# chenghuige/golden-huffman

Hardware: AMD Instinct MI355X
Metric: encode+decode GB/s (input bytes) (higher is better)
Workload: dtype u8

## Files before the change

### golden-huffman_amd/csrc/ghf_kernels.hip

```cpp
#include "ghf_device.h"

namespace ghf {

#define GHF_HADD(x, sh) atomicAdd(&lh[((((x) >> (sh)) & 0xFFu) << 5) | rep], 1u)

__device__ __forceinline__ void hist_vec(uint32_t* lh, uint32_t rep, const uint4& v) {
  GHF_HADD(v.x, 0); GHF_HADD(v.x, 8); GHF_HADD(v.x, 16); GHF_HADD(v.x, 24);
  GHF_HADD(v.y, 0); GHF_HADD(v.y, 8); GHF_HADD(v.y, 16); GHF_HADD(v.y, 24);
  GHF_HADD(v.z, 0); GHF_HADD(v.z, 8); GHF_HADD(v.z, 16); GHF_HADD(v.z, 24);
  GHF_HADD(v.w, 0); GHF_HADD(v.w, 8); GHF_HADD(v.w, 16); GHF_HADD(v.w, 24);
}

__global__ __launch_bounds__(kHistThreads) void k_histogram(const uint8_t* __restrict__ in, uint64_t n,
                                                            uint32_t chunk32, uint32_t nchunks,
                                                            uint32_t* __restrict__ chunk_hist,
                                                            unsigned long long* __restrict__ hist,
                                                            unsigned long long* __restrict__ acc ,
                                                            uint32_t add ) {
  static_assert(kHistRep == 32, "replica index is lane % 32");
  __shared__ uint32_t lh[256 * kHistRep];
  __shared__ bool s_last;
  const uint32_t tid = threadIdx.x;
  const uint32_t rep = tid & 31u;
  uint32_t prev = 0;
  unsigned long long total = 0;
  const uint64_t chunk = chunk32;
  const uint32_t V = chunk32 >> 12;
  const uint32_t nfullchunks = (uint32_t)(n / chunk);
  const bool fast = V >= 4u && (chunk32 & 4095u) == 0 && (((uintptr_t)in) & 15u) == 0 && nfullchunks > 0;
  auto vptr = [&](uint32_t c, uint32_t j) -> const uint4* {
    if (c >= nfullchunks) c = nfullchunks - 1;
    return reinterpret_cast<const uint4*>(in + (uint64_t)c * chunk) + (uint64_t)j * kHistThreads + tid;
  };
  uint4 A = make_uint4(0, 0, 0, 0), B = A;
  if (fast) {
    A = load_stream(vptr(blockIdx.x, 0));
    B = load_stream(vptr(blockIdx.x, 1));
  }
  for (uint32_t i = tid; i < 256 * kHistRep; i += kHistThreads) lh[i] = 0;
  __syncthreads();

  __shared__ uint32_t s_tick;
  auto finish_chunk = [&](uint32_t c) -> uint32_t {
    __syncthreads();
    const uint32_t posted = s_tick;
    uint32_t s = 0;
#pragma unroll
    for (uint32_t j = 0; j < kHistRep; ++j) s += lh[(tid << 5) | ((j + tid) & 31u)];
    const uint32_t cnt = s - prev;
    prev = s;
    chunk_hist[(uint64_t)c * 256 + tid] = cnt;
    total += cnt;
    __syncthreads();
    return posted;
  };

  if (fast) {
    const uint32_t ncls = gridDim.x < 16u ? 1u : (gridDim.x < 128u ? gridDim.x >> 3 : 16u);
    const uint32_t cls = (blockIdx.x >> 3) % ncls;
    unsigned long long* tick = acc + 32 * 256 + 16 + cls * 16;
    auto draw = [&]() -> uint32_t { return 2u * gridDim.x + (uint32_t)atomicAdd(tick, 1ull) * ncls + cls; };
    uint32_t cur = blockIdx.x;
    uint32_t nxt = blockIdx.x + gridDim.x;
    auto vat = [&](uint32_t g) -> const uint4* { return g < V ? vptr(cur, g) : vptr(nxt, g - V); };
    const uint32_t Vmain = V & ~3u, Vrest = V & 3u;
    while (cur < nfullchunks) {
      uint32_t t_next = 0;
      if (tid == 0) t_next = draw();
      for (uint32_t j = 0; j < Vmain; j += 4) {
        const uint4 C = load_stream(vat(j + 2)), D = load_stream(vat(j + 3));
        hist_vec(lh, rep, A);
        hist_vec(lh, rep, B);
        A = load_stream(vat(j + 4));
        B = load_stream(vat(j + 5));
        hist_vec(lh, rep, C);
        hist_vec(lh, rep, D);
      }
      if (Vrest == 1u) {
        hist_vec(lh, rep, A);
        A = B;
        B = load_stream(vptr(nxt, 1));
      } else if (Vrest == 2u) {
        hist_vec(lh, rep, A);
        hist_vec(lh, rep, B);
        A = load_stream(vptr(nxt, 0));
        B = load_stream(vptr(nxt, 1));
      } else if (Vrest == 3u) {
        const uint4 C = load_stream(vptr(cur, V - 1));
        hist_vec(lh, rep, A);
        hist_vec(lh, rep, B);
        A = load_stream(vptr(nxt, 0));
        B = load_stream(vptr(nxt, 1));
        hist_vec(lh, rep, C);
      }
      if (tid == 0) s_tick = t_next;
      const uint32_t posted = finish_chunk(cur);
      cur = nxt;
      nxt = posted;
    }
  }

  const uint32_t g0 = fast ? (blockIdx.x == 0 ? nfullchunks : nchunks) : blockIdx.x;
  const uint32_t gstep = fast ? nchunks : gridDim.x;
  for (uint32_t c = g0; c < nchunks; c += gstep) {
    const uint64_t base = (uint64_t)c * chunk;
    const uint64_t len = (n - base < chunk) ? (n - base) : chunk;
    const uint8_t* p = in + base;
    uint32_t head = (uint32_t)((16u - (uint32_t)((uintptr_t)p & 15u)) & 15u);
    if (head > len) head = (uint32_t)len;
    if (tid < head) atomicAdd(&lh[((uint32_t)p[tid] << 5) | rep], 1u);
    const uint4* pv = reinterpret_cast<const uint4*>(p + head);
    const uint64_t nvec = (len - head) >> 4;
    for (uint64_t i = tid; i < nvec; i += kHistThreads) {
      const uint4 v0 = pv[i];
      hist_vec(lh, rep, v0);
    }
    const uint64_t tail0 = head + (nvec << 4);
    if (tail0 + tid < len) atomicAdd(&lh[((uint32_t)p[tail0 + tid] << 5) | rep], 1u);
    (void)finish_chunk(c);
  }
  unsigned long long* rep_base = acc + (uint64_t)(blockIdx.x & 31u) * 256;
  if (total) atomicAdd(&rep_base[tid], total);
  asm volatile("s_waitcnt vmcnt(0)" ::: "memory");
  __syncthreads();
  if (tid == 0) {
    const unsigned long long t = atomicAdd(&acc[32 * 256], 1ull);
    s_last = (t + 1 == gridDim.x);
    if (s_last) __builtin_amdgcn_fence(__ATOMIC_ACQUIRE, "agent");
    asm volatile("s_waitcnt vmcnt(0)" ::: "memory");
  }
  __syncthreads();
  if (s_last) {
    unsigned long long part[32];
#pragma unroll
    for (int r = 0; r < 32; ++r) part[r] = __hip_atomic_load(&acc[r * 256 + tid], __ATOMIC_RELAXED, __HIP_MEMORY_SCOPE_AGENT);
    unsigned long long sum = 0;
#pragma unroll
    for (int r = 0; r < 32; ++r) {
      sum += part[r];
      __hip_atomic_store(&acc[r * 256 + tid], 0ull, __ATOMIC_RELAXED, __HIP_MEMORY_SCOPE_AGENT);
    }
    hist[tid] = add ? hist[tid] + sum : sum;
    if (tid < 16) __hip_atomic_store(&acc[32 * 256 + 16 + tid * 16], 0ull, __ATOMIC_RELAXED, __HIP_MEMORY_SCOPE_AGENT);
    if (tid == 0) {
      hist[256] = 1;
      __hip_atomic_store(&acc[32 * 256], 0ull, __ATOMIC_RELAXED, __HIP_MEMORY_SCOPE_AGENT);
    }
  }
}

void launch_histogram(const uint8_t* d_in, uint64_t n, uint32_t chunk, uint32_t nchunks, uint32_t* d_chunk_hist,
                      uint64_t* d_hist, uint64_t* d_acc, bool add, hipStream_t s) {
  static int ncu = 0;
  if (ncu == 0) {
    int dev = 0;
    hipDeviceProp_t prop;
    if (hipGetDevice(&dev) == hipSuccess && hipGetDeviceProperties(&prop, dev) == hipSuccess) ncu = prop.multiProcessorCount;
    if (ncu < 1) ncu = 256;
  }
  uint32_t grid = (uint32_t)(4 * ncu);
  if (grid > nchunks) grid = nchunks;
  if (grid == 0) grid = 1;
  hipLaunchKernelGGL(k_histogram, dim3(grid), dim3(kHistThreads), 0, s, d_in, n, chunk, nchunks, d_chunk_hist,
                     reinterpret_cast<unsigned long long*>(d_hist), reinterpret_cast<unsigned long long*>(d_acc),
                     add ? 1u : 0u);
}

struct HeapLds {
  alignas(16) unsigned long long slot[528];
  uint16_t parent[GHF_NSYM + 256 + 7];
  uint16_t cur[GHF_NSYM + 3];
};

typedef unsigned long long u64t;
struct alignas(16) U64x2 { u64t x, y; };

__device__ __forceinline__ bool heap_gt(u64t a, u64t b) { return a > (b | 511ull); }

__device__ __forceinline__ void heap_sift_up(HeapLds& h, int hole, u64t e) {
  while (hole > 0) {
    const int parent = (hole - 1) >> 1;
    const u64t pe = h.slot[parent + 1];
    if (!heap_gt(pe, e)) break;
    h.slot[hole + 1] = pe;
    hole = parent;
  }
  h.slot[hole + 1] = e;
}

__device__ __forceinline__ u64t heap_pop(HeapLds& h, int& n) {
  const u64t top = h.slot[1];
  const int len = n - 1;
  n = len;
  if (len < 1) return top;
  const u64t value = h.slot[len + 1];
  int hole = 0;
  const int lim = (len - 1) >> 1;
  while (hole < lim) {
    const U64x2 c = *reinterpret_cast<const U64x2*>(&h.slot[2 * hole + 2]);
    const U64x2 g0 = *reinterpret_cast<const U64x2*>(&h.slot[4 * hole + 4]);
    const U64x2 g1 = *reinterpret_cast<const U64x2*>(&h.slot[4 * hole + 6]);
    const bool left = heap_gt(c.y, c.x);
    const int child = 2 * hole + (left ? 1 : 2);
    h.slot[hole + 1] = left ? c.x : c.y;
    hole = child;
    if (hole < lim) {
      const U64x2 g = left ? g0 : g1;
      const bool left2 = heap_gt(g.y, g.x);
      const int child2 = 2 * hole + (left2 ? 1 : 2);
      h.slot[hole + 1] = left2 ? g.x : g.y;
      hole = child2;
    }
  }
  if ((len & 1) == 0 && hole == ((len - 2) >> 1)) {
    const int child = 2 * (hole + 1);
    h.slot[hole + 1] = h.slot[child];
    hole = child - 1;
  }
  heap_sift_up(h, hole, value);
  return top;
}

__device__ __forceinline__ u64t wave_uniform(u64t x) {
  const uint32_t lo = (uint32_t)__builtin_amdgcn_readfirstlane((int)(uint32_t)x);
  const uint32_t hi = (uint32_t)__builtin_amdgcn_readfirstlane((int)(uint32_t)(x >> 32));
  return ((u64t)hi << 32) | lo;
}

__device__ __forceinline__ u64t lane_above(u64t x) {
  const uint32_t lo = (uint32_t)__builtin_amdgcn_update_dpp(0, (int)(uint32_t)x, 0x101, 0xF, 0xF, false);
  const uint32_t hi = (uint32_t)__builtin_amdgcn_update_dpp(0, (int)(uint32_t)(x >> 32), 0x101, 0xF, 0xF, false);
  return ((u64t)hi << 32) | lo;
}

__device__ __forceinline__ u64t wave_heap_pop(HeapLds& h, int& n, int lane) {
  const int len = __builtin_amdgcn_readfirstlane(n) - 1;
  n = len;
  const uint32_t tA = lane ? (uint32_t)lane : 128u, tB = 64u + (uint32_t)lane;
  const U64x2 ca = *reinterpret_cast<const U64x2*>(&h.slot[2 * tA]);
  const U64x2 cb = *reinterpret_cast<const U64x2*>(&h.slot[2 * tB]);
  const u64t top_v = h.slot[1];
  const u64t value_v = h.slot[len + 1];
  __builtin_amdgcn_sched_barrier(0);
  const u64t top = wave_uniform(top_v);
  if (len < 1) return top;
  const u64t value = wave_uniform(value_v);
  const unsigned long long R0 = __ballot(!heap_gt(ca.y, ca.x));
  const unsigned long long R1 = __ballot(!heap_gt(cb.y, cb.x));
  const uint32_t lim = (uint32_t)(len - 1) >> 1;
  const int D = 31 - __clz(len);
  uint32_t t = 1;
  asm("s_bitcmp1_b64 %1, %0\n\ts_addc_u32 %0, %0, %0\n\t"
      "s_bitcmp1_b64 %1, %0\n\ts_addc_u32 %0, %0, %0\n\t"
      "s_bitcmp1_b64 %1, %0\n\ts_addc_u32 %0, %0, %0\n\t"
      "s_bitcmp1_b64 %1, %0\n\ts_addc_u32 %0, %0, %0\n\t"
      "s_bitcmp1_b64 %1, %0\n\ts_addc_u32 %0, %0, %0\n\t"
      "s_bitcmp1_b64 %1, %0\n\ts_addc_u32 %0, %0, %0\n\t"
      "s_bitcmp1_b64 %2, %0\n\ts_addc_u32 %0, %0, %0"
      : "+s"(t)
      : "s"(R0), "s"(R1)
      : "scc");
  const int steps = D - 1 > 0 ? D - 1 : 0;
  t >>= 7 - steps;
  if (t <= lim) t = 2u * t + (uint32_t)(((t < 64u || t == 128u ? R0 : R1) >> (t & 63u)) & 1ull);
  t <<= (((uint32_t)len & 1u) ^ 1u) & (uint32_t)(t == ((uint32_t)len >> 1));
  const int k = 31 - __clz(t);
  const uint32_t sh = (uint32_t)(k - lane) & 31u;
  const bool onp = lane < k;
  const uint32_t u = onp ? (t >> sh) : 1u;
  const U64x2 c = *reinterpret_cast<const U64x2*>(&h.slot[2 * u]);
  const u64t cv = ((t >> ((sh - 1u) & 31u)) & 1u) ? c.y : c.x;
  const unsigned long long S = __ballot(!heap_gt(cv, value)) & ((1ull << k) - 1ull);
  const int m = S ? 64 - __clzll((long long)S) : 0;
  if (lane <= m) h.slot[lane < m ? u : (t >> ((uint32_t)(k - m) & 31u))] = lane < m ? cv : value;
  wave_sync();
  return top;
}

struct PushLoad {
  u64t pe;
  int aj, depth;
  bool on;
};
__device__ __forceinline__ PushLoad wave_heap_push_load(const HeapLds& h, int n_, int lane) {
  const int n = __builtin_amdgcn_readfirstlane(n_);
  PushLoad L;
  L.depth = 31 - __clz(n + 1);
  L.on = lane >= 1 && lane <= L.depth;
  L.aj = ((n + 1) >> lane) - 1;
  L.pe = L.on ? h.slot[L.aj + 1] : 0ull;
  return L;
}
__device__ __forceinline__ void wave_heap_push_finish(HeapLds& h, const PushLoad& L, u64t e, int lane) {
  const bool stop = L.on && !heap_gt(L.pe, e);
  const unsigned long long sm = __ballot(stop);
  const int t = sm ? (__ffsll((long long)sm) - 1) - 1 : L.depth;
  const u64t up = lane_above(L.pe);
  if (lane <= t) h.slot[L.aj + 1] = (lane < t) ? up : e;
  wave_sync();
}
__device__ __forceinline__ void wave_heap_push(HeapLds& h, int n_, u64t e, int lane) {
  const PushLoad L = wave_heap_push_load(h, n_, lane);
  wave_heap_push_finish(h, L, e, lane);
}

struct CodeLds {
  uint32_t num[40];
  uint32_t first_code[64];
  uint32_t start_pos[64];
  int32_t min_len, max_len;
};

struct LimitLds {
  unsigned long long w[2][2 * GHF_NSYM];
  uint8_t is_leaf[33][2 * GHF_NSYM];
  uint16_t order[GHF_NSYM + 3];
  uint16_t len_of[34], taken[34];
  uint32_t newlen[GHF_NSYM + 3];
  long long freq[GHF_NSYM + 3];
  int n;
};

__device__ void limit_lengths_32(LimitLds& Q, const uint32_t (&len)[5], int lane) {
  constexpr int kLimit = 32;
  const long long* freq = Q.freq;
  if (lane == 0) Q.n = 0;
  __syncthreads();
#pragma unroll 1
  for (int j = 0; j < 5; ++j) {
    const int s = lane + 64 * j;
    if (s >= GHF_NSYM || len[j] == 0) continue;
    const long long f = freq[s];
    int rank = 0;
    for (int t = 0; t < GHF_NSYM; ++t) {
      const long long g = freq[t];
      rank += (g != 0) && (g < f || (g == f && t < s));
    }
    Q.order[rank] = (uint16_t)s;
    atomicAdd(&Q.n, 1);
  }
  __syncthreads();
  if (lane == 0) {
    const int n = Q.n;
    int prev_n = 0, cur = 0;
    for (int d = kLimit; d >= 1; --d) {
      const unsigned long long* pw = Q.w[cur ^ 1];
      unsigned long long* cw = Q.w[cur];
      const int npk = prev_n / 2;
      int li = 0, pi = 0, k = 0;
      while (li < n || pi < npk) {
        const unsigned long long lw = li < n ? (unsigned long long)freq[Q.order[li]] : ~0ull;
        const unsigned long long pk = pi < npk ? pw[2 * pi] + pw[2 * pi + 1] : ~0ull;
        if (li < n && (pi >= npk || lw <= pk)) {
          cw[k] = lw;
          Q.is_leaf[d][k] = 1;
          ++li;
        } else {
          cw[k] = pk;
          Q.is_leaf[d][k] = 0;
          ++pi;
        }
        ++k;
      }
      Q.len_of[d] = (uint16_t)k;
      prev_n = k;
      cur ^= 1;
    }
    int need = 2 * n - 2;
    for (int d = 1; d <= kLimit; ++d) {
      if (need > (int)Q.len_of[d]) need = Q.len_of[d];
      int leaves = 0;
      for (int k = 0; k < need; ++k) leaves += Q.is_leaf[d][k];
      Q.taken[d] = (uint16_t)leaves;
      need = 2 * (need - leaves);
    }
  }
  __syncthreads();
  for (int i = lane; i < GHF_NSYM; i += 64) Q.newlen[i] = 0;
  __syncthreads();
  for (int i = lane; i < Q.n; i += 64) {
    uint32_t l = 0;
    for (int d = 1; d <= kLimit; ++d) l += i < (int)Q.taken[d];
    Q.newlen[Q.order[i]] = l;
  }
  __syncthreads();
}

struct NoLimitLds {};
template <bool LIMIT>
__global__ __launch_bounds__(64) void k_build_code(const unsigned long long* __restrict__ hist, ghf_code* __restrict__ out,
                                                   int* __restrict__ status, uint32_t empty_ok) {
  __shared__ HeapLds heap;
  __shared__ typename std::conditional<LIMIT, LimitLds, NoLimitLds>::type Q;
  __builtin_amdgcn_s_setprio(3);
  __shared__ CodeLds cl;
  __shared__ int s_ndata;
  const int lane = threadIdx.x;
  long long fr[5];
#pragma unroll
  for (int j = 0; j < 5; ++j) {
    const int s = lane + 64 * j;
    fr[j] = s < GHF_NSYM ? (long long)hist[s] : 0ll;
    if constexpr (LIMIT) {
      if (s < GHF_NSYM) Q.freq[s] = fr[j];
    }
  }
  for (int s = lane; s < GHF_NSYM; s += 64) heap.cur[s] = (uint16_t)s;
  for (int i = lane; i < GHF_NSYM + 256 + 7; i += 64) heap.parent[i] = 0;
  if (lane < 40) cl.num[lane] = 0;
  cl.first_code[lane] = 0;
  cl.start_pos[lane] = 0;
  __syncthreads();

  {
    int n = 0, ndata = 0;
    for (int s = 0; s < GHF_NSYM; ++s) {
      const u64t f = (u64t)__shfl(fr[s >> 6], s & 63, 64);
      if (f) {
        wave_heap_push(heap, n, (f << 9) | (u64t)s, lane);
        ++n;
        if (s < 256) ++ndata;
      }
    }
    if (lane == 0) s_ndata = ndata;
    const int times = n - 1;
    for (int t = 0; t < times; ++t) {
      const u64t e1 = wave_heap_pop(heap, n, lane);
      const u64t e2 = wave_heap_pop(heap, n, lane);
      const int s1 = (int)(e1 & 511u), s2 = (int)(e2 & 511u);
      const int node = GHF_NSYM + t;
      const PushLoad pl = wave_heap_push_load(heap, n, lane);
      const uint16_t g1 = heap.cur[s1], g2 = heap.cur[s2];
      if (lane == 0) {
        heap.parent[g1] = (uint16_t)node;
        heap.parent[g2] = (uint16_t)node;
        heap.cur[s2] = (uint16_t)node;
      }
      const u64t f = (e1 >> 9) + (e2 >> 9);
      wave_heap_push_finish(heap, pl, (f << 9) | (u64t)s2, lane);
      ++n;
    }
  }
  __syncthreads();
  if (s_ndata == 0 && !empty_ok) {
    if (lane == 0) latch_status(status, GHF_E_EMPTY);
    return;
  }
  uint32_t len[5], node[5];
#pragma unroll
  for (int j = 0; j < 5; ++j) {
    len[j] = 0;
    node[j] = (uint32_t)(lane + 64 * j);
    if (node[j] >= GHF_NSYM) node[j] = GHF_NSYM + 256 + 1;
  }
  for (int step = 0; step < 256; ++step) {
    bool any = false;
#pragma unroll
    for (int j = 0; j < 5; ++j) {
      const uint32_t p = heap.parent[node[j]];
      if (p) {
        node[j] = p;
        len[j] += 1;
        any = true;
      }
    }
    if (!__ballot(any)) break;
  }
  if (s_ndata == 0 && lane == 0) len[4] = 1;
  uint32_t mx = 0;
#pragma unroll
  for (int j = 0; j < 5; ++j) {
    if (lane + 64 * j >= GHF_NSYM) len[j] = 0;
    mx = len[j] > mx ? len[j] : mx;
  }
#pragma unroll
  for (int d = 32; d >= 1; d >>= 1) {
    const uint32_t o = __shfl_xor(mx, d, 64);
    mx = o > mx ? o : mx;
  }
  int max_len = (int)mx;
  if (max_len > 32) {
    if constexpr (!LIMIT) {
      if (lane == 0) latch_status(status, GHF_E_CODELEN);
      return;
    } else {
      limit_lengths_32(Q, len, lane);
      mx = 0;
#pragma unroll
      for (int j = 0; j < 5; ++j) {
        const int s = lane + 64 * j;
        len[j] = s < GHF_NSYM ? Q.newlen[s] : 0u;
        mx = len[j] > mx ? len[j] : mx;
      }
#pragma unroll
      for (int d = 32; d >= 1; d >>= 1) {
        const uint32_t o = __shfl_xor(mx, d, 64);
        mx = o > mx ? o : mx;
      }
      max_len = (int)mx;
    }
  }

#pragma unroll
  for (int j = 0; j < 5; ++j) {
    const int s = lane + 64 * j;
    if (s < GHF_NSYM) {
      out->length[s] = len[j];
      out->codeword[s] = 0;
      out->symbol[s] = 0xFFFFFFFFu;
      if (len[j]) atomicAdd(&cl.num[len[j]], 1u);
    }
  }
  __syncthreads();
  const uint32_t num = (lane >= 1 && lane <= max_len) ? cl.num[lane] : 0u;
  const unsigned long long nzmask = __ballot(num != 0);
  const int min_len = __ffsll((long long)nzmask) - 1;
  const uint32_t spos = wave_incl_scan_u32(num) - num;
  if (lane >= 1 && lane <= max_len) cl.start_pos[lane] = spos;
  if (lane == 0) {
    uint32_t fc = 0;
    cl.first_code[max_len] = 0;
    for (int i = max_len - 1; i >= 1; --i) {
      fc = (fc + cl.num[i + 1]) >> 1;
      cl.first_code[i] = fc;
    }
    for (int i = 1; i < min_len; ++i) cl.first_code[i] = 1024;
    out->min_len = min_len;
    out->max_len = max_len;
  }
  __syncthreads();
  out->first_code[lane] = cl.first_code[lane];
  out->start_pos[lane] = cl.start_pos[lane];
  uint32_t seen = 0;
  for (int j = 0; j < 5; ++j) {
    for (int L = min_len; L <= max_len; ++L) {
      const bool m = (len[j] == (uint32_t)L);
      const unsigned long long mask = __ballot(m);
      if (mask == 0) continue;
      const uint32_t before = __shfl(seen, L, 64);
      if (m) {
        const uint32_t r = before + (uint32_t)__popcll(mask & ((1ull << lane) - 1ull));
        const int s = lane + 64 * j;
        out->codeword[s] = cl.first_code[L] + r;
        out->symbol[cl.start_pos[L] + r] = (uint32_t)s;
      }
      if (lane == L) seen += (uint32_t)__popcll(mask);
    }
  }
}

void launch_build_code(const uint64_t* d_hist, ghf_code* d_code, int* d_status, uint32_t flags, hipStream_t s) {
  if (flags & GHF_CODE_LIMIT)
    hipLaunchKernelGGL(k_build_code<true>, dim3(1), dim3(64), 0, s, reinterpret_cast<const unsigned long long*>(d_hist), d_code, d_status,
                       flags & GHF_EMPTY_OK);
  else
    hipLaunchKernelGGL(k_build_code<false>, dim3(1), dim3(64), 0, s, reinterpret_cast<const unsigned long long*>(d_hist), d_code, d_status,
                       flags & GHF_EMPTY_OK);
}

struct TreeLds {
  uint16_t tl[256], tr[256];
  uint16_t size[GHF_NSYM + 256 + 7];
  uint8_t is_right[GHF_NSYM + 256 + 7];
  uint32_t code_hi[256];
  uint32_t max_len, min_len;
  int n;
};

__global__ __launch_bounds__(64) void k_crs_build_code(const unsigned long long* __restrict__ hist, ghf_tree* __restrict__ out_tree,
                                                       ghf_code* __restrict__ out_code, unsigned long long* __restrict__ start_bit,
                                                       int* __restrict__ status) {
  __shared__ HeapLds heap;
  __shared__ TreeLds T;
  __shared__ ghf_tree tree;
  __builtin_amdgcn_s_setprio(3);
  const int lane = threadIdx.x;
  for (int s = lane; s < GHF_NSYM; s += 64) heap.cur[s] = (uint16_t)s;
  for (int i = lane; i < GHF_NSYM + 256 + 7; i += 64) {
    heap.parent[i] = 0;
    T.size[i] = 1;
    T.is_right[i] = 0;
  }
  for (int i = lane; i < (int)(sizeof(ghf_tree) / 4); i += 64) reinterpret_cast<uint32_t*>(&tree)[i] = 0;
  if (lane == 0) {
    T.max_len = 0;
    T.min_len = 0xFFFFFFFFu;
  }
  __syncthreads();
  int n = 0;
  for (int s = 0; s < 256; ++s) {
    const u64t f = wave_uniform((u64t)hist[s]);
    if (f) {
      wave_heap_push(heap, n, (f << 9) | (u64t)s, lane);
      ++n;
    }
  }
  const int nleaves = n;
  if (nleaves < 2) {
    if (lane == 0) latch_status(status, nleaves == 0 ? GHF_E_EMPTY : GHF_E_SINGLE);
    return;
  }
  const int times = n - 1;
  for (int t = 0; t < times; ++t) {
    const u64t e1 = wave_heap_pop(heap, n, lane);
    const u64t e2 = wave_heap_pop(heap, n, lane);
    const int s1 = (int)(e1 & 511u), s2 = (int)(e2 & 511u);
    const int node = GHF_NSYM + t;
    if (lane == 0) {
      const int a = heap.cur[s1], b = heap.cur[s2];
      heap.parent[a] = (uint16_t)node;
      heap.parent[b] = (uint16_t)node;
      T.tl[t] = (uint16_t)a;
      T.tr[t] = (uint16_t)b;
      T.is_right[b] = 1;
      T.size[node] = (uint16_t)(1 + T.size[a] + T.size[b]);
      heap.cur[s2] = (uint16_t)node;
    }
    wave_heap_push(heap, n, (((e1 >> 9) + (e2 >> 9)) << 9) | (u64t)s2, lane);
    ++n;
  }
  __syncthreads();
  for (int v = lane; v < GHF_NSYM + times; v += 64) {
    const bool leaf = v < 256;
    if (v == 256 || (leaf && heap.parent[v] == 0)) continue;
    uint32_t len = 0, pre = 0;
    unsigned long long code = 0;
    int x = v;
    for (int p; (p = heap.parent[x]) != 0; x = p) {
      const uint32_t r = T.is_right[x];
      if (len < 64) code |= (unsigned long long)r << len;
      ++len;
      pre += 1u + (r ? (uint32_t)T.size[T.tl[p - GHF_NSYM]] : 0u);
    }
    if (leaf) {
      tree.header[2 * pre] = 0;
      tree.header[2 * pre + 1] = (uint8_t)v;
      atomicMax(&T.max_len, len);
      atomicMin(&T.min_len, len);
      if (len <= 64) {
        out_code->length[v] = len;
        out_code->codeword[v] = (uint32_t)code;
        T.code_hi[v] = (uint32_t)(code >> 32);
      }
    } else {
      tree.header[2 * pre] = 255;
      tree.header[2 * pre + 1] = 255;
      const int t = v - GHF_NSYM;
      const int a = T.tl[t], b = T.tr[t];
      tree.left[t] = (uint16_t)(a < GHF_NSYM ? a : 256 + (a - GHF_NSYM));
      tree.right[t] = (uint16_t)(b < GHF_NSYM ? b : 256 + (b - GHF_NSYM));
    }
  }
  __syncthreads();
  const bool deep = T.max_len > 32u;
  for (int s = lane; s < GHF_NSYM; s += 64) {
    const bool absent = s == 256 || heap.parent[s] == 0;
    if (absent) {
      out_code->length[s] = 0;
      out_code->codeword[s] = 0;
    }
    out_code->symbol[s] = deep ? (absent ? 0u : T.code_hi[s]) : 0xFFFFFFFFu;
  }
  for (int i = lane; i < 64; i += 64) {
    out_code->first_code[i] = 0;
    out_code->start_pos[i] = 0;
  }
  if (T.max_len > 64u) {
    if (lane == 0) latch_status(status, GHF_E_CODELEN);
    return;
  }
  if (lane == 0) {
    tree.root = (uint32_t)(256 + times - 1);
    tree.n_leaves = (uint32_t)nleaves;
    tree.max_len = T.max_len;
    tree.tree_bytes = 2u * (2u * (uint32_t)nleaves - 1u);
    out_code->min_len = (int32_t)T.min_len;
    out_code->max_len = (int32_t)T.max_len;
    if (start_bit) *start_bit = 8ull * ((unsigned long long)tree.tree_bytes + 2ull);
  }
  __syncthreads();
  for (int i = lane; i < (int)(sizeof(ghf_tree) / 4); i += 64)
    reinterpret_cast<uint32_t*>(out_tree)[i] = reinterpret_cast<const uint32_t*>(&tree)[i];
}

void launch_crs_build_code(const uint64_t* d_hist, ghf_tree* d_tree, ghf_code* d_code, uint64_t* d_start_bit, int* d_status,
                           hipStream_t s) {
  hipLaunchKernelGGL(k_crs_build_code, dim3(1), dim3(64), 0, s, reinterpret_cast<const unsigned long long*>(d_hist), d_tree,
                     d_code, reinterpret_cast<unsigned long long*>(d_start_bit), d_status);
}

__global__ __launch_bounds__(256) void k_crs_finish(const ghf_tree* __restrict__ tree, const unsigned long long* __restrict__ total_bits,
                                                    uint8_t* __restrict__ out, unsigned long long* __restrict__ out_bytes,
                                                    const int* __restrict__ status) {
  if (*status != 0) return;
  const uint32_t tb = tree->tree_bytes;
  for (uint32_t i = threadIdx.x; i < tb; i += 256) out[i] = tree->header[i];
  if (threadIdx.x == 0) {
    const unsigned long long t = *total_bits;
    const unsigned long long whole = t >> 3;
    const uint32_t left = (uint32_t)((8u - (uint32_t)(t & 7u)) & 7u);
    out[tb] = (uint8_t)left;
    out[tb + 1] = left ? out[tb + 2 + whole] : (uint8_t)0;
    if (out_bytes) *out_bytes = (unsigned long long)tb + 2ull + whole;
  }
}

void launch_crs_finish(const ghf_tree* d_tree, const uint64_t* d_total_bits, uint8_t* d_out, uint64_t* d_out_bytes, int* d_status,
                       hipStream_t s) {
  hipLaunchKernelGGL(k_crs_finish, dim3(1), dim3(256), 0, s, d_tree, reinterpret_cast<const unsigned long long*>(d_total_bits), d_out,
                     reinterpret_cast<unsigned long long*>(d_out_bytes), d_status);
}

__global__ __launch_bounds__(256) void k_write_header(const ghf_code* __restrict__ code, uint8_t* __restrict__ out,
                                                      uint64_t cap, int* __restrict__ status) {
  const int max_len = code->max_len;
  if (max_len < 1 || max_len > 32) return;
  const int nwords = 1 + GHF_NSYM + 2 + 2 * max_len;
  if ((uint64_t)nwords * 4 > cap) {
    if (threadIdx.x == 0) latch_status(status, GHF_E_CAP);
    return;
  }
  uint32_t* o = reinterpret_cast<uint32_t*>(out);
  for (int w = threadIdx.x; w < nwords; w += blockDim.x) o[w] = bswap32(header_word(code, w, max_len));
}

void launch_write_header(const ghf_code* d_code, uint8_t* d_out, uint64_t cap, int* d_status, hipStream_t s) {
  hipLaunchKernelGGL(k_write_header, dim3(1), dim3(256), 0, s, d_code, d_out, cap, d_status);
}

__global__ __launch_bounds__(256) void k_chunk_bits(const uint32_t* __restrict__ chunk_hist, uint32_t nchunks,
                                                    const ghf_code* __restrict__ code, uint64_t* __restrict__ bits) {
  const int lane = threadIdx.x & 63;
  const uint32_t wave = (blockIdx.x * blockDim.x + threadIdx.x) >> 6;
  const uint32_t nwaves = (gridDim.x * blockDim.x) >> 6;
  const uint4 L = reinterpret_cast<const uint4*>(code->length)[lane];
  for (uint32_t c = wave; c < nchunks; c += nwaves) {
    const uint4 h = reinterpret_cast<const uint4*>(chunk_hist + (uint64_t)c * 256)[lane];
    unsigned long long b = (unsigned long long)h.x * L.x + (unsigned long long)h.y * L.y +
                           (unsigned long long)h.z * L.z + (unsigned long long)h.w * L.w;
#pragma unroll
    for (int d = 32; d >= 1; d >>= 1) b += __shfl_xor(b, d, 64);
    if (lane == 0) bits[c] = b;
  }
}

__global__ __launch_bounds__(256) void k_chunk_bits_direct(const uint8_t* __restrict__ in, uint64_t n, uint32_t chunk32,
                                                           uint32_t nchunks, const ghf_code* __restrict__ code,
                                                           uint64_t* __restrict__ bits) {
  __shared__ uint32_t ll[256];
  ll[threadIdx.x] = code->length[threadIdx.x];
  __syncthreads();
  const int lane = threadIdx.x & 63;
  const uint32_t wave = (blockIdx.x * blockDim.x + threadIdx.x) >> 6;
  const uint32_t nwaves = (gridDim.x * blockDim.x) >> 6;
  const uint64_t chunk = chunk32;
  for (uint32_t c = wave; c < nchunks; c += nwaves) {
    const uint64_t base = (uint64_t)c * chunk;
    const uint64_t len = (n - base < chunk) ? (n - base) : chunk;
    unsigned long long b = 0;
    const uint8_t* p = in + base;
    uint64_t head = (16u - (uint32_t)((uintptr_t)p & 15u)) & 15u;
    if (head > len) head = len;
    if ((uint64_t)lane < head) b += ll[p[lane]];
    const uint4* pv = reinterpret_cast<const uint4*>(p + head);
    const uint64_t nvec = (len - head) >> 4;
    uint32_t acc = 0;
    for (uint64_t i = lane; i < nvec; i += 64) {
      const uint4 v = pv[i];
      const uint32_t w[4] = {v.x, v.y, v.z, v.w};
#pragma unroll
      for (int k = 0; k < 4; ++k)
        acc += ll[w[k] & 0xFFu] + ll[(w[k] >> 8) & 0xFFu] + ll[(w[k] >> 16) & 0xFFu] + ll[w[k] >> 24];
      if ((i >> 6) % 4096u == 4095u) {
        b += acc;
        acc = 0;
      }
    }
    b += acc;
    const uint64_t tail0 = head + (nvec << 4);
    if (tail0 + (uint64_t)lane < len) b += ll[p[tail0 + lane]];
#pragma unroll
    for (int d = 32; d >= 1; d >>= 1) b += __shfl_xor(b, d, 64);
    if (lane == 0) bits[c] = b;
  }
}

__global__ __launch_bounds__(1024) void k_scan(uint64_t* __restrict__ v, uint32_t count, uint64_t* __restrict__ total_out) {
  __shared__ unsigned long long wsum[16];
  const int tid = threadIdx.x, lane = tid & 63, w = tid >> 6;
  const uint32_t ipt = (count + 1023u) / 1024u;
  const uint32_t lo = tid * ipt;
  const uint32_t hi = (lo + ipt < count) ? lo + ipt : count;
  unsigned long long mine = 0;
  const bool small = ipt <= 8u;
  unsigned long long x8[8];
  if (small) {
#pragma unroll
    for (uint32_t k = 0; k < 8; ++k) {
      const uint32_t i = lo + k;
      x8[k] = (k < ipt && i < hi) ? v[i] : 0ull;
    }
#pragma unroll
    for (uint32_t k = 0; k < 8; ++k) mine += x8[k];
  } else {
    for (uint32_t i = lo; i < hi; ++i) mine += v[i];
  }
  unsigned long long s = mine;
#pragma unroll
  for (int d = 1; d < 64; d <<= 1) {
    const unsigned long long t = __shfl_up(s, d, 64);
    if (lane >= d) s += t;
  }
  if (lane == 63) wsum[w] = s;
  __syncthreads();
  unsigned long long woff = 0, total = 0;
  for (int k = 0; k < 16; ++k) {
    const unsigned long long x = wsum[k];
    if (k < w) woff += x;
    total += x;
  }
  unsigned long long run = woff + s - mine;
  if (small) {
#pragma unroll
    for (uint32_t k = 0; k < 8; ++k) {
      const uint32_t i = lo + k;
      if (k < ipt && i < hi) v[i] = run;
      run += x8[k];
    }
  } else {
    for (uint32_t i = lo; i < hi; ++i) {
      const unsigned long long x = v[i];
      v[i] = run;
      run += x;
    }
  }
  if (tid == 0) {
    v[count] = total;
    if (total_out) *total_out = total;
  }
}

void launch_scan(uint64_t* d_v, uint32_t count, uint64_t* d_total, hipStream_t s) {
  hipLaunchKernelGGL(k_scan, dim3(1), dim3(1024), 0, s, d_v, count, d_total);
}

void launch_plan(const uint8_t* d_in, uint64_t n, uint32_t chunk, uint32_t nchunks, const uint32_t* d_chunk_hist,
                 const ghf_code* d_code, uint64_t* d_chunk_off, uint64_t* d_total_bits, hipStream_t s) {
  uint32_t blocks = (nchunks + 3) / 4;
  if (blocks > 2048) blocks = 2048;
  if (blocks == 0) blocks = 1;
  if (d_chunk_hist)
    hipLaunchKernelGGL(k_chunk_bits, dim3(blocks), dim3(256), 0, s, d_chunk_hist, nchunks, d_code, d_chunk_off);
  else
    hipLaunchKernelGGL(k_chunk_bits_direct, dim3(blocks), dim3(256), 0, s, d_in, n, chunk, nchunks, d_code,
                       d_chunk_off);
  hipLaunchKernelGGL(k_scan, dim3(1), dim3(1024), 0, s, d_chunk_off, nchunks, d_total_bits);
}

__global__ void k_store_u64(uint64_t* dst, const uint64_t* src, uint64_t add) { *dst = (src ? *src : 0ull) + add; }
void launch_store_u64(uint64_t* d_dst, const uint64_t* d_src_opt, uint64_t add, hipStream_t s) {
  hipLaunchKernelGGL(k_store_u64, dim3(1), dim3(1), 0, s, d_dst, d_src_opt, add);
}

__global__ void k_load_u16(uint64_t* dst, const uint16_t* src) { *dst = *src; }
void launch_load_u16(uint64_t* d_dst, const uint16_t* d_src, hipStream_t s) { hipLaunchKernelGGL(k_load_u16, dim3(1), dim3(1), 0, s, d_dst, d_src); }

__global__ void k_shard_start(const ghf_code* code, const uint64_t* totals, int rank, uint64_t* start_bit) {
  uint64_t b = 8ull * (1040ull + 8ull * (uint64_t)code->max_len);
  for (int r = 0; r < rank; ++r) b += totals[r];
  *start_bit = b;
}
void launch_shard_start(const ghf_code* d_code, const uint64_t* d_totals, int rank, uint64_t* d_start_bit, hipStream_t s) {
  hipLaunchKernelGGL(k_shard_start, dim3(1), dim3(1), 0, s, d_code, d_totals, rank, d_start_bit);
}

template <bool NT>
__global__ __launch_bounds__(256) void k_stream_copy(const uint4* __restrict__ src, uint4* __restrict__ dst, uint64_t nvec) {
  const uint64_t per = (nvec + gridDim.x - 1) / gridDim.x;
  const uint64_t lo = (uint64_t)blockIdx.x * per;
  const uint64_t end = lo + per < nvec ? lo + per : nvec;
  uint64_t i = lo + threadIdx.x;
  auto ld = [&](uint64_t k) -> uint4 { return NT ? load_stream(src + k) : src[k]; };
  auto st = [&](uint64_t k, const uint4& v) {
    if (NT) store_stream(dst + k, v);
    else dst[k] = v;
  };
  for (; i + 3 * 256 < end; i += 4 * 256) {
    const uint4 a = ld(i), b = ld(i + 256), c = ld(i + 512), d = ld(i + 768);
    st(i, a); st(i + 256, b); st(i + 512, c); st(i + 768, d);
  }
  for (; i < end; i += 256) st(i, ld(i));
}
__global__ void k_tail_copy(const uint8_t* src, uint8_t* dst, uint64_t from, uint64_t n) {
  const uint64_t i = from + threadIdx.x;
  if (i < n) dst[i] = src[i];
}
void launch_stream_copy(const uint8_t* d_src, uint8_t* d_dst, uint64_t n, bool nt, hipStream_t s) {
  const uint64_t nvec = n / 16;
  if (nvec) {
    uint64_t blocks = (nvec + 255) / 256;
    if (blocks > 4096) blocks = 4096;
    if (nt) hipLaunchKernelGGL(k_stream_copy<true>, dim3((uint32_t)blocks), dim3(256), 0, s, reinterpret_cast<const uint4*>(d_src), reinterpret_cast<uint4*>(d_dst), nvec);
    else hipLaunchKernelGGL(k_stream_copy<false>, dim3((uint32_t)blocks), dim3(256), 0, s, reinterpret_cast<const uint4*>(d_src), reinterpret_cast<uint4*>(d_dst), nvec);
  }
  if (n & 15) hipLaunchKernelGGL(k_tail_copy, dim3(1), dim3(16), 0, s, d_src, d_dst, nvec * 16, n);
}

}
```

Before: 965.8.

## Double-buffer histogram counts in 16-bit halves to drop a barrier per chunk

Each shared-memory histogram word now holds two 16-bit counters. Consecutive chunks alternate halves, so finish_chunk reads one half and clears it with atomicAnd while the next chunk accumulates into the other half. This removes the trailing __syncthreads and the running-prefix subtraction. The main loop also keeps four vectors in flight with sched_barrier fences, and the remainder cases are specialized at compile time. In exchange it adds an atomicAnd per replica and relies on a static_assert that a chunk's counts fit in 16 bits.

Result: no change. 962.4 (-0.4%).

```diff
diff --git a/golden-huffman_amd/csrc/ghf_kernels.hip b/golden-huffman_amd/csrc/ghf_kernels.hip
--- a/golden-huffman_amd/csrc/ghf_kernels.hip
+++ b/golden-huffman_amd/csrc/ghf_kernels.hip
@@ -2,14 +2,20 @@
 
 namespace ghf {
 
-#define GHF_HADD(x, sh) atomicAdd(&lh[((((x) >> (sh)) & 0xFFu) << 5) | rep], 1u)
-
-__device__ __forceinline__ void hist_vec(uint32_t* lh, uint32_t rep, const uint4& v) {
+static_assert(kMaxChunk / kHistRep + 2 * (kHistThreads / kHistRep) < 65536, "a chunk's counts must fit a 16-bit half");
+
+#define GHF_HADD(x, sh) atomicAdd(&lh[((((x) >> (sh)) & 0xFFu) << 5) | rep], inc)
+
+__device__ __forceinline__ void hist_vec(uint32_t* lh, uint32_t rep, uint32_t inc, const uint4& v) {
   GHF_HADD(v.x, 0); GHF_HADD(v.x, 8); GHF_HADD(v.x, 16); GHF_HADD(v.x, 24);
   GHF_HADD(v.y, 0); GHF_HADD(v.y, 8); GHF_HADD(v.y, 16); GHF_HADD(v.y, 24);
   GHF_HADD(v.z, 0); GHF_HADD(v.z, 8); GHF_HADD(v.z, 16); GHF_HADD(v.z, 24);
   GHF_HADD(v.w, 0); GHF_HADD(v.w, 8); GHF_HADD(v.w, 16); GHF_HADD(v.w, 24);
 }
+
+#define GHF_HFENCE() __builtin_amdgcn_sched_barrier(0)
+
+template <uint32_t N> struct HistRest { static constexpr uint32_t value = N; };
 
 __global__ __launch_bounds__(kHistThreads) void k_histogram(const uint8_t* __restrict__ in, uint64_t n,
                                                             uint32_t chunk32, uint32_t nchunks,
@@ -22,7 +28,7 @@
   __shared__ bool s_last;
   const uint32_t tid = threadIdx.x;
   const uint32_t rep = tid & 31u;
-  uint32_t prev = 0;
+  uint32_t half = 0;
   unsigned long long total = 0;
   const uint64_t chunk = chunk32;
   const uint32_t V = chunk32 >> 12;
@@ -32,71 +38,85 @@
     if (c >= nfullchunks) c = nfullchunks - 1;
     return reinterpret_cast<const uint4*>(in + (uint64_t)c * chunk) + (uint64_t)j * kHistThreads + tid;
   };
-  uint4 A = make_uint4(0, 0, 0, 0), B = A;
+  uint4 A = make_uint4(0, 0, 0, 0), B = A, C = A, D = A;
   if (fast) {
     A = load_stream(vptr(blockIdx.x, 0));
     B = load_stream(vptr(blockIdx.x, 1));
+    C = load_stream(vptr(blockIdx.x, 2));
+    D = load_stream(vptr(blockIdx.x, 3));
   }
   for (uint32_t i = tid; i < 256 * kHistRep; i += kHistThreads) lh[i] = 0;
   __syncthreads();
 
-  __shared__ uint32_t s_tick;
+  __shared__ uint32_t s_tick[2];
   auto finish_chunk = [&](uint32_t c) -> uint32_t {
     __syncthreads();
-    const uint32_t posted = s_tick;
+    const uint32_t posted = __builtin_amdgcn_readfirstlane(s_tick[half >> 4]);
+    const uint32_t keep = 0xFFFF0000u >> half;
     uint32_t s = 0;
 #pragma unroll
-    for (uint32_t j = 0; j < kHistRep; ++j) s += lh[(tid << 5) | ((j + tid) & 31u)];
-    const uint32_t cnt = s - prev;
-    prev = s;
-    chunk_hist[(uint64_t)c * 256 + tid] = cnt;
-    total += cnt;
-    __syncthreads();
+    for (uint32_t j = 0; j < kHistRep; ++j) {
+      uint32_t* p = &lh[(tid << 5) | ((j + tid) & 31u)];
+      s += (__hip_atomic_load(p, __ATOMIC_RELAXED, __HIP_MEMORY_SCOPE_WORKGROUP) >> half) & 0xFFFFu;
+      atomicAnd(p, keep);
+    }
+    chunk_hist[(uint64_t)c * 256 + tid] = s;
+    total += s;
+    half ^= 16u;
     return posted;
   };
 
   if (fast) {
     const uint32_t ncls = gridDim.x < 16u ? 1u : (gridDim.x < 128u ? gridDim.x >> 3 : 16u);
     const uint32_t cls = (blockIdx.x >> 3) % ncls;
-    unsigned long long* tick = acc + 32 * 256 + 16 + cls * 16;
-    auto draw = [&]() -> uint32_t { return 2u * gridDim.x + (uint32_t)atomicAdd(tick, 1ull) * ncls + cls; };
-    uint32_t cur = blockIdx.x;
-    uint32_t nxt = blockIdx.x + gridDim.x;
-    auto vat = [&](uint32_t g) -> const uint4* { return g < V ? vptr(cur, g) : vptr(nxt, g - V); };
-    const uint32_t Vmain = V & ~3u, Vrest = V & 3u;
-    while (cur < nfullchunks) {
-      uint32_t t_next = 0;
-      if (tid == 0) t_next = draw();
-      for (uint32_t j = 0; j < Vmain; j += 4) {
-        const uint4 C = load_stream(vat(j + 2)), D = load_stream(vat(j + 3));
-        hist_vec(lh, rep, A);
-        hist_vec(lh, rep, B);
-        A = load_stream(vat(j + 4));
-        B = load_stream(vat(j + 5));
-        hist_vec(lh, rep, C);
-        hist_vec(lh, rep, D);
+    uint32_t* tick = reinterpret_cast<uint32_t*>(acc + 32 * 256 + 16 + cls * 16);
+    const uint32_t Vmain = V & ~3u;
+    auto fast_chunks = [&](auto rest) {
+      constexpr uint32_t R = decltype(rest)::value;
+      uint32_t cur = blockIdx.x;
+      uint32_t nxt = blockIdx.x + gridDim.x;
+      auto vat = [&](uint32_t j, uint32_t k) -> const uint4* {
+        return j + 4 < Vmain ? vptr(cur, j + 4 + k) : vptr(nxt, k);
+      };
+      uint4 E0 = A, E1 = A, E2 = A;
+      while (cur < nfullchunks) {
+        uint32_t drawn = 0;
+        if (tid == 0) drawn = atomicAdd(tick, 1u);
+        const uint32_t inc = 1u << half;
+        if (R >= 1u) E0 = load_stream(vptr(cur, Vmain));
+        if (R >= 2u) E1 = load_stream(vptr(cur, Vmain + 1));
+        if (R >= 3u) E2 = load_stream(vptr(cur, Vmain + 2));
+        GHF_HFENCE();
+        uint32_t j = 0;
+        do {
+          hist_vec(lh, rep, inc, A);
+          hist_vec(lh, rep, inc, B);
+          GHF_HFENCE();
+          A = load_stream(vat(j, 0));
+          B = load_stream(vat(j, 1));
+          GHF_HFENCE();
+          hist_vec(lh, rep, inc, C);
+          hist_vec(lh, rep, inc, D);
+          GHF_HFENCE();
+          C = load_stream(vat(j, 2));
+          D = load_stream(vat(j, 3));
+          GHF_HFENCE();
+          j += 4;
+        } while (j < Vmain);
+        if (R >= 1u) hist_vec(lh, rep, inc, E0);
+        if (R >= 2u) hist_vec(lh, rep, inc, E1);
+        if (R >= 3u) hist_vec(lh, rep, inc, E2);
+        if (tid == 0) s_tick[half >> 4] = 2u * gridDim.x + drawn * ncls + cls;
+        const uint32_t posted = finish_chunk(cur);
+        cur = nxt;
+        nxt = posted;
       }
-      if (Vrest == 1u) {
-        hist_vec(lh, rep, A);
-        A = B;
-        B = load_stream(vptr(nxt, 1));
-      } else if (Vrest == 2u) {
-        hist_vec(lh, rep, A);
-        hist_vec(lh, rep, B);
-        A = load_stream(vptr(nxt, 0));
-        B = load_stream(vptr(nxt, 1));
-      } else if (Vrest == 3u) {
-        const uint4 C = load_stream(vptr(cur, V - 1));
-        hist_vec(lh, rep, A);
-        hist_vec(lh, rep, B);
-        A = load_stream(vptr(nxt, 0));
-        B = load_stream(vptr(nxt, 1));
-        hist_vec(lh, rep, C);
-      }
-      if (tid == 0) s_tick = t_next;
-      const uint32_t posted = finish_chunk(cur);
-      cur = nxt;
-      nxt = posted;
+    };
+    switch (V & 3u) {
+      case 0: fast_chunks(HistRest<0>()); break;
+      case 1: fast_chunks(HistRest<1>()); break;
+      case 2: fast_chunks(HistRest<2>()); break;
+      default: fast_chunks(HistRest<3>()); break;
     }
   }
 
@@ -108,19 +128,21 @@
     const uint8_t* p = in + base;
     uint32_t head = (uint32_t)((16u - (uint32_t)((uintptr_t)p & 15u)) & 15u);
     if (head > len) head = (uint32_t)len;
-    if (tid < head) atomicAdd(&lh[((uint32_t)p[tid] << 5) | rep], 1u);
+    const uint32_t inc = 1u << half;
+    if (tid < head) atomicAdd(&lh[((uint32_t)p[tid] << 5) | rep], inc);
     const uint4* pv = reinterpret_cast<const uint4*>(p + head);
     const uint64_t nvec = (len - head) >> 4;
     for (uint64_t i = tid; i < nvec; i += kHistThreads) {
       const uint4 v0 = pv[i];
-      hist_vec(lh, rep, v0);
+      hist_vec(lh, rep, inc, v0);
     }
     const uint64_t tail0 = head + (nvec << 4);
-    if (tail0 + tid < len) atomicAdd(&lh[((uint32_t)p[tail0 + tid] << 5) | rep], 1u);
+    if (tail0 + tid < len) atomicAdd(&lh[((uint32_t)p[tail0 + tid] << 5) | rep], inc);
     (void)finish_chunk(c);
   }
   unsigned long long* rep_base = acc + (uint64_t)(blockIdx.x & 31u) * 256;
   if (total) atomicAdd(&rep_base[tid], total);
+  __builtin_amdgcn_s_waitcnt(0x0F70);
   asm volatile("s_waitcnt vmcnt(0)" ::: "memory");
   __syncthreads();
   if (tid == 0) {
```
